# bolcom/serenade

Hardware: AMD Instinct MI355X
Metric: predict_next queries/sec (higher is better)
Workload: dtype u32 ids / i32 accumulators / f64 scores; 1 GPU; BASELINE configs[2]: synthetic 60000000 interactions / 1760000 items, k=1500 m=2500 idf_weighting=2 last_items=4 how_many=21; batch_per_gpu=1048576, query_pool_batches=2, parallelism=query-sharded replicas x1 (no data-path collective), index=csr (built by this library)

## Files before the change

### serenade_amd/csrc/srn_fast.hip

```cpp
#include <hip/hip_runtime.h>

#include <cstdio>
#include <cstdlib>

#include "srn_device.h"
#include "srn_prep.h"
#include "srn_kernels.h"

namespace srn {

#ifndef SRN_FAST_NT
#define SRN_FAST_NT 1
#endif
typedef uint32_t fin_v4u __attribute__((ext_vector_type(4)));
__device__ __forceinline__ void fin_store(uint4* p, const uint4& v) {
#if SRN_FAST_NT
    __builtin_nontemporal_store((fin_v4u{v.x, v.y, v.z, v.w}), reinterpret_cast<fin_v4u*>(p));
#else
    *p = v;
#endif
}
__device__ __forceinline__ uint4 fin_load(const uint4* p) {
#if SRN_FAST_NT
    const fin_v4u v = __builtin_nontemporal_load(reinterpret_cast<const fin_v4u*>(p)); return make_uint4(v.x, v.y, v.z, v.w);
// ... 141 lines not shown
#define SRN_MERGE_ODD 1
#endif
    const uint32_t sb = sa + la, total = la + lb, g = ((total + (1u << lg_nthr) - 1u) >> lg_nthr) | (SRN_MERGE_ODD ? 1u : 0u);
    const uint32_t d0 = min(ttid * g, total), d1 = min(d0 + g, total);
    if (d0 >= d1) return;
    uint32_t lo = d0 > lb ? d0 - lb : 0u, hi = min(d0, la);
    while (lo < hi) {
        const uint32_t mid = (lo + hi) >> 1;
        if (in[sa + mid] > in[sb + d0 - 1 - mid]) lo = mid + 1; else hi = mid;
    }
    const uint32_t* pa = in + sa + lo; const uint32_t* pb = in + sb + (d0 - lo);
    const uint32_t* const ea = in + sb; const uint32_t* const eb = in + sb + lb;
    uint32_t va = pa < ea ? *pa : 0u, vb = pb < eb ? *pb : 0u;
    uint32_t* c = out + sa + d0; uint32_t* const ce = out + sa + d1;
    for (; c < ce; ++c) {
        const bool ta = va > vb;
        *c = max(va, vb);
        const uint32_t* q = (ta ? pa : pb) + 1;
        pa = ta ? q : pa; pb = ta ? pb : q;
        const uint32_t nxt = *q;
        const uint32_t nv = q < (ta ? ea : eb) ? nxt : 0u;
        va = ta ? nv : va; vb = ta ? vb : nv;
    }
}

#ifndef SRN_FAST_FUSED_CUT
#define SRN_FAST_FUSED_CUT 1
#endif
template <int G>
__device__ __forceinline__ uint32_t fast_cut(const uint32_t* F, uint32_t* nbl, uint32_t n, uint32_t NB, uint32_t m, uint32_t k, const uint8_t* wlut, uint32_t* misc, uint32_t tid, uint32_t lane) {
    constexpr int BLOCK = 512;
    const uint32_t NBM = (1u << NB) - 1u;
    const uint32_t g = (n + BLOCK - 1) / BLOCK, o0 = min(tid * g, n), o1 = min(o0 + g, n);
    uint32_t fv[G + 3];
#pragma unroll
    for (int x = 0; x < G + 3; ++x) fv[x] = F[min(o0 + (uint32_t)x, n - 1u)];
    const uint32_t prev0 = o0 > 0u && o0 < o1 ? F[o0 - 1u] >> NB : 0xFFFFFFFFu;
#pragma unroll
    for (int x = 0; x < G + 3; ++x) fv[x] = o0 + (uint32_t)x < n ? fv[x] : 0u;
    {
        uint32_t carry = 0u, carry_r = 0xFFFFFFFFu;
#pragma unroll
        for (int x = G + 2; x >= 0; --x) { const uint32_t r = fv[x] >> NB; carry = r == carry_r ? carry | fv[x] : fv[x]; carry_r = r; fv[x] = carry; }
    }
    uint32_t fmask = 0u, firsts = 0u;
    {
        uint32_t prev = prev0;
#pragma unroll
        for (int x = 0; x < G; ++x) { const bool in = o0 + (uint32_t)x < o1; const uint32_t r = fv[x] >> NB; const bool f1 = in && r != prev; fmask |= f1 ? 1u << x : 0u; firsts += f1; prev = in ? r : prev; }
    }
    uint32_t Call;
    const uint32_t idx0 = block_excl_scan<BLOCK>(firsts, misc + FS_SCAN_A, Call);
    const uint32_t Cm = min(Call, m);
    if (Cm <= k) {
        uint32_t idx = idx0;
#pragma unroll
        for (int x = 0; x < G; ++x) if ((fmask >> x) & 1u) { if (idx < m) nbl[idx] = fv[x]; ++idx; }
        return Cm;
    }
    uint32_t inm = 0u; unsigned long long nmp = 0ull, acc = 0ull;
    {
        uint32_t idx = idx0, nmv[G];
#pragma unroll
        for (int x = 0; x < G; ++x) nmv[x] = (uint32_t)wlut[fv[x] & NBM];
#pragma unroll
        for (int x = 0; x < G; ++x) {
            const bool f1 = (fmask >> x) & 1u, in = f1 && idx < m;
            idx += f1;
            inm |= in ? 1u << x : 0u;
            nmp |= in ? (unsigned long long)nmv[x] << (4 * x) : 0ull;
            acc += in ? 1ull << (4u * nmv[x]) : 0ull;
        }
    }
    uint32_t* cls = misc + FS_CLS;
    {
        uint32_t tot[8];
#pragma unroll
        for (int jj = 0; jj < 4; ++jj) {
            const unsigned long long t = (acc >> (4 * jj)) & 0x000F000F000F000Full;
            tot[2 * jj] = wave_sum((uint32_t)t); tot[2 * jj + 1] = wave_sum((uint32_t)(t >> 32));
        }
        const uint32_t dw = (lane & 3u) * 2u + (lane >> 3);
        uint32_t pick = tot[0];
#pragma unroll
        for (int x = 1; x < 8; ++x) pick = dw == (uint32_t)x ? tot[x] : pick;
        const uint32_t mycnt = lane < 16u ? (pick >> (16u * ((lane >> 2) & 1u))) & 0xFFFFu : 0u;
        if (mycnt) atomicAdd(&cls[lane], mycnt);
    }
    __syncthreads();
    uint32_t nstar, rstar;
    {
        const uint32_t cv = lane < 16u ? cls[lane] : 0u; const uint32_t pre = wave_incl_scan(cv);
        const uint32_t suf = (uint32_t)__builtin_amdgcn_readlane((int)pre, 63) - pre + cv;
        const unsigned long long reach = __ballot(suf >= k);
        nstar = 63u - (uint32_t)__clzll((long long)reach);
        rstar = k - ((uint32_t)__builtin_amdgcn_readlane((int)suf, (int)nstar) - (uint32_t)__builtin_amdgcn_readlane((int)cv, (int)nstar));
    }
    uint32_t mine = 0;
#pragma unroll
    for (int x = 0; x < G; ++x) mine += ((inm >> x) & 1u) && (uint32_t)((nmp >> (4 * x)) & 15ull) == nstar;
    uint32_t tot_star;
    uint32_t before = block_excl_scan<BLOCK>(mine, misc + FS_SCAN_B, tot_star);
    uint32_t sel = 0, tmask = 0;
#pragma unroll
    for (int x = 0; x < G; ++x) {
        const bool in = (inm >> x) & 1u; const uint32_t c = (uint32_t)((nmp >> (4 * x)) & 15ull);
        const bool eq = in && c == nstar, take = in && (c > nstar || (eq && before < rstar));
        tmask |= take ? 1u << x : 0u; sel += take; before += eq;
    }
    const uint32_t inc = wave_incl_scan(sel);
    uint32_t base = 0; if (lane == 63u && inc) base = atomicAdd(&misc[FS_NB], inc);
    uint32_t at = (uint32_t)__builtin_amdgcn_readlane((int)base, 63) + inc - sel;
#pragma unroll
    for (int x = 0; x < G; ++x) if ((tmask >> x) & 1u) nbl[at++] = fv[x];
    return 0xFFFFFFFFu;
}

enum { FM_FUSED = 0, FM_FRONT = 1, FM_BACK = 2 };
template <int WG_PER_CU, bool FRAG, bool WIDE, int MODE = FM_FUSED, bool MID = false, bool BIG = false, bool LONG = false, bool TINY = false>
#ifndef SRN_FAST_WAVES
#define SRN_FAST_WAVES (WG_PER_CU * 2)
#endif
#ifndef SRN_TINY_WAVES
#define SRN_TINY_WAVES 2
#endif
__global__ __launch_bounds__(512, TINY ? SRN_TINY_WAVES : BIG ? 4 : SRN_FAST_WAVES) void vmis_fast_kernel(DeviceIndex ix_arg, LaunchParams p_arg, FastParams f_arg) {
#if SRN_FAST_SMALL
    static_assert(!BIG || MID, "BIG is a form of MID"); static_assert(!LONG || BIG, "LONG is a form of BIG");
    constexpr uint32_t SIDF = BIG ? F_BIG_TOTAL - (F_TOTAL - F_SIDF) : F_SIDF, SATTR = SIDF + 512 * 8;
    constexpr uint32_t MW = (SIDF - F_WORK) / 4;
    __shared__ __attribute__((aligned(16))) char smem[BIG ? F_BIG_TOTAL : F_TOTAL];
#else
    extern __shared__ __attribute__((aligned(16))) char smem[];
#endif
    typedef const __attribute__((address_space(4))) char* KArg;
    const KArg ka = (KArg)__builtin_amdgcn_kernarg_segment_ptr();
    constexpr size_t OFF_P = (sizeof(DeviceIndex) + alignof(LaunchParams) - 1) / alignof(LaunchParams) * alignof(LaunchParams);
    constexpr size_t OFF_F = (OFF_P + sizeof(LaunchParams) + alignof(FastParams) - 1) / alignof(FastParams) * alignof(FastParams);
    const __attribute__((address_space(4))) DeviceIndex& ix = *(const __attribute__((address_space(4))) DeviceIndex*)ka;
    const __attribute__((address_space(4))) LaunchParams& p = *(const __attribute__((address_space(4))) LaunchParams*)(ka + OFF_P);
    const __attribute__((address_space(4))) FastParams& f = *(const __attribute__((address_space(4))) FastParams*)(ka + OFF_F);
    constexpr int BLOCK = 512, NW = 8;
    constexpr int NL = LONG ? (int)F_LONG_LISTS : MID ? (int)F_MID_LISTS : 4;
    constexpr uint32_t SINV = F_SINV;
    static_assert(!MID || MODE == FM_FUSED, "MID: fused form only");
    const uint32_t tid = threadIdx.x, lane = tid & 63u, wave = tid >> 6;
    const unsigned long long lt = (1ull << lane) - 1ull;
    static_assert(!TINY || (MODE == FM_FUSED && !BIG && !FRAG), "TINY: the lean or the MID fused form over an unsharded index");
    if constexpr (TINY) {
        unsigned long long* const a_items = reinterpret_cast<unsigned long long*>(smem + F_W10 + 64); uint32_t* const a_off = reinterpret_cast<uint32_t*>(smem + F_W10 + 64 + 64);
        const uint32_t alen = f.tiny_len;
        if (f.serve == nullptr) {
        if (alen) { if (tid < 8u) a_items[tid] = f.tiny_items[tid]; if (tid == 0u) { a_off[0] = 0u; a_off[1] = alen; } __syncthreads(); }
        if (tid < PREP_LANES) prep_group(ix_arg, alen ? (const uint64_t*)a_items : p.items_flat, alen ? (const uint32_t*)a_off : p.q_off, alen ? 0u : blockIdx.x, tid, p.m, p.max_len,
                                         const_cast<char*>(p.prep) + (size_t)blockIdx.x * p.prep_stride, nullptr, 0u, nullptr);
        __syncthreads();
        }
    }

    uint32_t* misc = (uint32_t*)(smem + F_MISC);
    uint8_t* wlut = (uint8_t*)(smem + F_WLUT);
    uint16_t* w10t = (uint16_t*)(smem + F_W10);
    uint32_t* nbl = (uint32_t*)(smem + F_NBL);
    unsigned long long* ckey = (unsigned long long*)(smem + F_CAND);
    uint32_t* cidx = (uint32_t*)(smem + F_CAND + F_CAND_CAP * 8);
    char* const acc_base = smem + F_HOT;
    uint32_t* hot = (uint32_t*)(smem + F_HOT);
    uint32_t* ikeys = (uint32_t*)(smem + F_TABLE);
    int* iacc = (int*)(smem + F_TABLE + F_TABLE_WORDS * 4);
    uint2* hits = (uint2*)(smem + F_HITS);
    uint32_t* surv = (uint32_t*)(smem + F_SURV);
    constexpr uint32_t SURV_CAP = F_SURV_WORDS - 256u;
    uint32_t* const cls_area = BIG ? (uint32_t*)(smem + SIDF) - 256 : surv + SURV_CAP;
    uint32_t* const dn_area = cls_area - F_M_MAX / 4u;
    uint2* const nb2 = reinterpret_cast<uint2*>(dn_area - F_K_MAX * 2u);
    uint32_t* thist = surv + SURV_CAP;
    auto num_of = [&](uint32_t set) -> uint32_t {
        if constexpr (MID) return (uint32_t)wlut[set & 31u] + (uint32_t)wlut[32u + (set >> 5)];
        else return (uint32_t)wlut[set]; };
    auto w10_of = [&](uint32_t set) -> uint32_t {
        if constexpr (MID) { const uint32_t lo = set & 31u, hi = set >> 5; const uint32_t mp = lo ? (uint32_t)wlut[64u + lo] : (uint32_t)wlut[96u + hi]; return (9u - mp) * ((uint32_t)wlut[lo] + (uint32_t)wlut[32u + hi]); }
        else return (uint32_t)w10t[set]; };

    unsigned long long* tacc = (unsigned long long*)(smem + F_MISC + FS_TACC * 4);
    if (tid < 16u) tacc[tid] = 0ull;
    const bool ticking = p.phase_cycles != nullptr;
    const bool business = (p.flags & SRN_FLAG_BUSINESS_LOGIC) != 0u;
    const uint32_t n_kept = ix.n_kept;
    auto qpos = [&](uint32_t pq) -> uint32_t { return ((wave + NW * (pq >> 6)) << 6) + (pq & 63u); };

    uint32_t* const pre = (uint32_t*)(smem + F_W10 + 64);
    bool have_pre = false;
    { const ItemMeta m0 = f.meta_sample[tid];
      ((double*)(smem + SIDF))[tid] = m0.idf > 0.0 ? m0.idf : 1.0; ((uint8_t*)(smem + SATTR))[tid] = (uint8_t)m0.attr;
      if (tid < 16u) ((double*)(smem + SINV))[tid] = tid < 8u ? f.inv_idf_hot[tid] : f.inv_idf_hi; }
    const bool listed = !MID && MODE == FM_BACK && f.mid_list != nullptr;
    const uint32_t q_end = TINY ? p.nq : LONG ? *f.long_cnt : BIG ? *f.bigq_cnt : MID || listed ? *f.mid_cnt : p.nq;
    const bool ordered = !MID && MODE != FM_FRONT && f.order != nullptr && !listed;
    const uint32_t ox = blockIdx.x & 7u;
    const bool serving = TINY && f.serve != nullptr;
    const uint32_t qi_step = serving ? 0u : ordered ? gridDim.x >> 3 : gridDim.x;
    uint32_t serve_seq = 0u; bool serve_have = false; unsigned long long serve_t0 = 0ull, serve_c0 = 0ull;
    if constexpr (TINY) { if (serving) serve_seq = __atomic_load_n(&(f.serve + blockIdx.x)->done_seq, __ATOMIC_RELAXED); }
    const uint32_t qi_end = ordered ? ord_count(f.order_dups != nullptr ? p.nq - *f.order_dups : p.nq, ox) : q_end;
    for (uint32_t qi = ordered ? blockIdx.x >> 3 : (MODE == FM_FRONT ? f.q_base : 0u) + blockIdx.x; qi < qi_end; qi += qi_step) {
        if constexpr (TINY) {
            if (serving) {
                uint32_t* const sv_flag = reinterpret_cast<uint32_t*>(smem + F_W10 + 64 + 192);
                unsigned long long* const sv_items = reinterpret_cast<unsigned long long*>(smem + F_W10 + 64); uint32_t* const sv_off = reinterpret_cast<uint32_t*>(smem + F_W10 + 64 + 128);
                ServeCtl* const c = f.serve + blockIdx.x;
                __syncthreads();
                if (wave == 0u) {
                    __threadfence_system();
                    uint32_t leave = 0u;
                    if (serve_have && lane == 0u) {
                        const uint32_t cnt = __atomic_load_n(&p.out_counts[blockIdx.x], __ATOMIC_RELAXED);
                        if (cnt & 0x80000000u) { (void)atomicExch(&f.slow_cnt[SC_GENERAL], 0u); (void)atomicExch(&f.slow_cnt[SC_MID], 0u); (void)atomicExch(&f.slow_cnt[SC_BIG_TICKET_LO], 0u); (void)atomicExch(&f.slow_cnt[SC_BIG_TICKET_HI], 0u); }
                        const unsigned long long t_end = wall_clock64();
                        c->stamp[2] = (uint32_t)(t_end - serve_t0); c->stamp[3] = (uint32_t)((unsigned long long)clock64() - serve_c0);
                        __atomic_store_n(&c->count, cnt, __ATOMIC_RELAXED);
                        __atomic_store_n(&c->status, (cnt & 0x80000000u) ? 1u : 0u, __ATOMIC_RELAXED);
                        __threadfence_system();
                        __atomic_store_n(&c->done_seq, serve_seq, __ATOMIC_RELAXED);
                    }
                    const unsigned long long t0 = wall_clock64(), idle = __builtin_nontemporal_load(&c->idle_ticks);
                    uint32_t w = 0u, s_new = 0u, n = 0u;
                    for (;;) {
                        if (lane < 16u) w = __atomic_load_n(reinterpret_cast<const uint32_t*>(c) + lane, __ATOMIC_RELAXED);
                        s_new = (uint32_t)__builtin_amdgcn_readlane((int)w, 0); n = min((uint32_t)__builtin_amdgcn_readlane((int)w, 1), 16u);
                        if (s_new != serve_seq) {
                            uint32_t x = lane >= 4u && lane < 4u + 2u * min(n, 5u) ? w : 0u;
#pragma unroll
                            for (int d = 1; d < 16; d <<= 1) x ^= __shfl_xor(x, d, 16);
                            if ((uint32_t)__builtin_amdgcn_readlane((int)x, 0) == ((uint32_t)__builtin_amdgcn_readlane((int)w, 2) ^ s_new ^ n)) break;
                        }
                        if ((uint32_t)__builtin_amdgcn_readlane((int)w, 3) != 0u || wall_clock64() - t0 > idle) { leave = 1u; break; }
                    }
                    if (!leave) {
                        serve_seq = s_new; serve_have = true; serve_t0 = wall_clock64(); serve_c0 = (unsigned long long)clock64();
                        if (lane >= 4u && lane < 14u) reinterpret_cast<uint32_t*>(sv_items)[lane - 4u] = w;
                        if (n > 5u && lane < 2u * (n - 5u)) reinterpret_cast<uint32_t*>(sv_items)[10u + lane] = __atomic_load_n(reinterpret_cast<const uint32_t*>(c->more) + lane, __ATOMIC_RELAXED);
                        if (lane == 0u) { sv_off[0] = 0u; sv_off[1] = n; p.out_counts[blockIdx.x] = 0x80000002u; c->stamp[0] = (uint32_t)(serve_t0 - t0); }
                    }
                    if (lane == 0u) sv_flag[0] = leave;
                }
                __syncthreads();
                if (sv_flag[0] != 0u) break;
                if (tid < PREP_LANES) prep_group(ix_arg, (const uint64_t*)sv_items, (const uint32_t*)sv_off, 0u, tid, p.m, p.max_len, const_cast<char*>(p.prep) + (size_t)blockIdx.x * p.prep_stride, nullptr, 0u, nullptr);
                __syncthreads();
                if (tid == 0u) c->stamp[1] = (uint32_t)(wall_clock64() - serve_t0);
            }
        }
        const uint32_t q = TINY ? qi : LONG ? f.long_list[qi] : BIG ? f.bigq_list[qi] : MID || listed ? f.mid_list[qi] : ordered ? (uint32_t)f.order[ord_pos(ox, qi)] : qi;
        const uint32_t q_ord_next = ordered && qi + qi_step < qi_end ? (uint32_t)f.order[ord_pos(ox, qi + qi_step)]
                                  : listed && qi + qi_step < qi_end ? f.mid_list[qi + qi_step] : 0xFFFFFFFFu;
#ifndef SRN_MID_PREFETCH
#define SRN_MID_PREFETCH 0
#endif
        const uint32_t q_after = !(MID && SRN_MID_PREFETCH) ? 0xFFFFFFFFu : qi + gridDim.x < q_end ? (BIG ? f.bigq_list : f.mid_list)[qi + gridDim.x] : 0xFFFFFFFFu;
        long long t_prev = ticking ? clock64() : 0;
        FAST_PRIO(FP_REC);
        const char* const rec = p.prep + (size_t)q * p.prep_stride;
        struct { uint32_t U, rmax, xlo, sumw, L, n_staged, cur_attr, unsafe; } hd;
        constexpr uint32_t HW = (uint32_t)sizeof(PrepHead) / 4u;
        struct { uint32_t idx, kept; unsigned long long base; } x0{kNone, 0u, 0ull};
        if (have_pre) {
            auto uni = [&](uint32_t w) -> uint32_t { return (uint32_t)__builtin_amdgcn_readfirstlane((int)pre[w]); };
            hd.U = uni(0); hd.rmax = uni(1); hd.xlo = uni(2); hd.sumw = uni(3); hd.L = uni(6); hd.n_staged = uni(7); hd.cur_attr = uni(16); hd.unsafe = uni(17);
            if (lane < (LONG ? 32u : MID ? 16u : 8u) && lane < hd.L) { const uint32_t* it = pre + HW + 6u * lane; x0.idx = it[0]; x0.kept = it[3]; x0.base = ((unsigned long long)it[5] << 32) | it[4]; }
        } else {
            const PrepHead h0 = *(const PrepHead*)rec;
            hd.U = h0.U; hd.rmax = h0.rmax; hd.xlo = h0.xlo; hd.sumw = h0.sumw; hd.L = h0.L; hd.n_staged = h0.n_staged; hd.cur_attr = h0.cur_attr; hd.unsafe = h0.unsafe;
            if ((MID ? lane < (LONG ? 32u : 16u) && lane < p.max_len : lane < 8u) && lane < hd.L) { const PrepItem pi = ((const PrepItem*)(rec + sizeof(PrepHead)))[lane]; x0.idx = pi.idx; x0.kept = pi.kept; x0.base = pi.base; }
        }
        have_pre = false;
        const uint32_t L = hd.L, n = hd.n_staged, U = hd.U;
        unsigned long long rm = __ballot(x0.kept > 0u);
#ifdef SRN_FAST_EXP_ONELIST
        rm &= 0ull - rm;
#endif
        const uint32_t nr = (uint32_t)__popcll(rm);
        const bool rel = MID || (WIDE && nr > 3u);
        const uint32_t NB = LONG ? F_LONG_NB : MID ? max(nr, 4u) : WIDE && !rel ? 3u : 4u, NBM = (1u << NB) - 1u, base = rel ? hd.xlo : 0u;
        const bool fits = hd.unsafe != 0u ? false : LONG ? L >= 1u && L <= F_LONG_LMAX && L <= p.max_len && hd.sumw <= F_LONG_CLASSES && nr <= F_LONG_LISTS && 2u * n + 8u + F_LONG_RES_WORDS <= MW && hd.rmax - hd.xlo < (1u << (32u - F_LONG_NB))
                        : MID ? L >= 1u && L <= F_MID_LMAX && L <= p.max_len && hd.sumw <= F_MID_CLASSES && nr <= F_MID_LISTS && 2u * n + 8u + 256u <= MW && hd.rmax - hd.xlo < (1u << (32u - NB))
                              : L >= 1u && L <= 8u && L <= p.max_len && hd.sumw <= 15u && nr <= 4u && 2u * n + 8u <= MW && (!rel || hd.rmax - hd.xlo < (1u << 28));
        uint32_t* const xq = MODE == FM_FUSED ? nullptr : f.xchg + (size_t)q * f.xchg_stride;
        if (!fits) {
            if constexpr (MODE == FM_FRONT) { if (tid == 0) xq[0] = 0xFFFFFFFFu; }
            else if (tid == 0) {
                if (hd.unsafe != 0u) f.slow_list[atomicAdd(&f.slow_cnt[SC_GENERAL], 1u)] = q;
                else if (!MID && MODE == FM_FUSED && f.bigq_list != nullptr && L >= 1u && L <= 8u && L <= p.max_len && hd.sumw <= 15u && nr <= 4u && hd.rmax - hd.xlo < (1u << 28) &&
                    2u * n + 8u + 256u <= (F_BIG_TOTAL - (F_TOTAL - F_SIDF) - F_WORK) / 4u) f.bigq_list[atomicAdd(f.bigq_cnt, 1u)] = q;
                else if (!MID && MODE == FM_FUSED && f.mid_list != nullptr && L >= 1u && L <= F_MID_LMAX && L <= p.max_len) f.mid_list[atomicAdd(f.mid_cnt, 1u)] = q;
                else if (!MID && MODE == FM_FUSED && f.long_list != nullptr && L > F_MID_LMAX && L <= F_LONG_LMAX && L <= p.max_len) f.long_list[atomicAdd(f.long_cnt, 1u)] = q;
                else if (MID && !BIG && f.bigq_list != nullptr && L >= 1u && L <= F_MID_LMAX && L <= p.max_len && hd.sumw <= F_MID_CLASSES && nr <= F_MID_LISTS && hd.rmax - hd.xlo < (1u << (32u - NB)) &&
                         2u * n + 8u + 256u <= (F_BIG_TOTAL - (F_TOTAL - F_SIDF) - F_WORK) / 4u) f.bigq_list[atomicAdd(f.bigq_cnt, 1u)] = q;
                else f.slow_list[atomicAdd(&f.slow_cnt[SC_GENERAL], 1u)] = q;
            }
            continue;
        }
        if (n == 0u) { if (tid == 0) { if constexpr (MODE == FM_FRONT) xq[0] = 0u; else p.out_counts[q] = 0u; } continue; }
        uint32_t kp[NL], ps[NL]; const uint32_t* src[NL];
#pragma unroll
        for (int r = 0; r < NL; ++r) {
            const int l = rm ? __ffsll((long long)rm) - 1 : 0;
            kp[r] = rm ? (uint32_t)__builtin_amdgcn_readlane((int)x0.kept, l) : 0u;
            const uint32_t blo = (uint32_t)__builtin_amdgcn_readlane((int)(uint32_t)x0.base, l), bhi = (uint32_t)__builtin_amdgcn_readlane((int)(uint32_t)(x0.base >> 32), l);
            src[r] = ix.post_rank + (((unsigned long long)bhi << 32) | blo);
            ps[r] = (uint32_t)l;
            rm &= rm - 1ull;
        }
        const uint32_t cur_idx = (uint32_t)__builtin_amdgcn_readlane((int)x0.idx, 0);
        const uint32_t cur_attr = hd.cur_attr;
        const uint32_t s1 = kp[0], s2 = s1 + kp[1], s3 = s2 + kp[2];

        uint32_t v[4][5];
        uint32_t K = 0;
        uint32_t pfv[4] = {0u, 0u, 0u, 0u};
        uint32_t xsv[3] = {0u, 0u, 0u};
        if constexpr (MODE == FM_BACK) {
            const uint32_t kv = xq[0];
#pragma unroll
            for (int t = 0; t < 3; ++t) xsv[t] = xq[1u + min(wave * 64u + lane + (uint32_t)t * BLOCK, f.xchg_stride - 2u)];
            K = (uint32_t)__builtin_amdgcn_readfirstlane((int)kv);
        } else {
#pragma unroll
        for (int r = 0; r < 4; ++r)
#pragma unroll
            for (int j = 0; j < 5; ++j) { v[r][j] = 0u; if ((uint32_t)j * BLOCK < kp[r]) v[r][j] = src[r][min(tid + j * BLOCK, kp[r] - 1u)]; }
        }
        __syncthreads();
        FAST_PRIO(FP_FRONT);
        if constexpr (MODE != FM_BACK) {
#pragma unroll
        for (int r = 0; r < 4; ++r)
#pragma unroll
            for (int j = 0; j < 5; ++j) asm volatile("" : "+v"(v[r][j]));
        }
        FAST_TICK(0);
        if (tid < (uint32_t)FS_TACC) misc[tid] = 0;
#ifndef SRN_FAST_EARLY_CLEAR
#define SRN_FAST_EARLY_CLEAR 0
#endif
        const uint32_t clr_lo = (!SRN_FAST_EARLY_CLEAR || MODE == FM_FRONT) ? F_TABLE : (MODE == FM_BACK || nr <= 1u) ? F_HOT : min(F_TABLE, max(F_HOT, (F_WORK + (2u * n + 16u) * 4u + 15u) & ~15u));
        if (SRN_FAST_EARLY_CLEAR && MODE != FM_FRONT) {
            uint4* z = reinterpret_cast<uint4*>(smem);
            for (uint32_t i = clr_lo / 16u + tid; i < F_TABLE / 16u; i += BLOCK) z[i] = make_uint4(0u, 0u, 0u, 0u);
        }
        if constexpr (LONG) {
            if (tid < 32u) {
                uint32_t pr = 0u;
#pragma unroll
                for (int r = 0; r < NL; ++r) pr = tid == (uint32_t)(31 - r) ? ps[r] : pr;
                wlut[tid] = (uint8_t)(L - pr); wlut[32u + tid] = (uint8_t)pr;
            }
        } else
        if constexpr (MID) {
            if (tid < 64u) {
                const uint32_t half = tid >> 5, hs = tid & 31u;
                uint32_t num = 0u, mp = 0u;
                const uint32_t lo = hs ? (uint32_t)__ffs((int)hs) - 1u : 0u;
#pragma unroll
                for (int r = 0; r < 5; ++r) { const uint32_t pr = half ? ps[5 + r] : ps[r]; num += ((hs >> r) & 1u) ? L - pr : 0u; mp = lo == (uint32_t)r ? pr : mp; }
                wlut[tid] = (uint8_t)num; wlut[64u + tid] = (uint8_t)mp;
            }
        } else
        if (tid < (1u << nr)) {
            const uint32_t num = ((tid & 1u) ? L - ps[0] : 0u) + ((tid & 2u) ? L - ps[1] : 0u) + ((tid & 4u) ? L - ps[2] : 0u) + ((tid & 8u) ? L - ps[3] : 0u);
            const uint32_t lo = tid ? (uint32_t)__ffs((int)tid) - 1u : 0u;
            const uint32_t mp = lo == 0u ? ps[0] : lo == 1u ? ps[1] : lo == 2u ? ps[2] : ps[3];
            wlut[tid] = (uint8_t)num; w10t[tid] = (uint16_t)((9u - mp) * num);
        }
        if constexpr (MODE == FM_BACK) {
            if (K == 0xFFFFFFFFu) { if (tid == 0) f.slow_list[atomicAdd(&f.slow_cnt[SC_GENERAL], 1u)] = q; continue; }
            if (K == 0u) { if (tid == 0) p.out_counts[q] = 0u; continue; }
        } else
        if (nr == 1u) {
            K = min(kp[0], p.k);
#pragma unroll
            for (int j = 0; j < 3; ++j) { const uint32_t e = tid + j * BLOCK; if ((uint32_t)j * BLOCK < K && e < K) {
                if constexpr (LONG) nb2[e] = make_uint2(((v[0][j] - base) << NB) | 31u, (uint32_t)((9 - (int)ps[0]) * (int)(L - ps[0])));
                else nbl[e] = ((v[0][j] - base) << NB) | 1u; } }
            __syncthreads();
            FAST_TICK(1);
        } else {
        uint32_t* const B1 = (uint32_t*)(smem + F_WORK); uint32_t* const B0 = B1 + n;
        static_assert(F_WORK == F_NBL, "the m-cut writes the neighbour list in place");
        if constexpr (MID) {
            const uint32_t nlev = nr <= 2u ? 1u : nr <= 4u ? 2u : nr <= 8u ? 3u : nr <= 16u ? 4u : 5u;
            uint32_t* const X = (nlev & 1u) ? B1 : B0; uint32_t* const Y = (nlev & 1u) ? B0 : B1;
            uint32_t pre_r[NL];
            { uint32_t a = 0u;
#pragma unroll
              for (int r = 0; r < NL; ++r) { pre_r[r] = a; a += kp[r]; } }
#pragma unroll
            for (int r = 0; r < 4; ++r)
#pragma unroll
                for (int j = 0; j < 5; ++j) { const uint32_t e = tid + j * BLOCK; if ((uint32_t)j * BLOCK < kp[r] && e < kp[r]) X[pre_r[r] + e] = ((v[r][j] - base) << NB) | (LONG ? 31u - (uint32_t)r : 1u << r); }
#pragma unroll
            for (int b4 = 4; b4 < NL; b4 += 4) {
                if (nr > (uint32_t)b4) {
                    constexpr int R4 = 4;
#pragma unroll
                    for (int r = 0; r < R4; ++r)
#pragma unroll
                        for (int j = 0; j < 5; ++j) { v[r][j] = 0u; if (b4 + r < NL) { if ((uint32_t)j * BLOCK < kp[b4 + r < NL ? b4 + r : 0]) v[r][j] = src[b4 + r < NL ? b4 + r : 0][min(tid + j * BLOCK, kp[b4 + r < NL ? b4 + r : 0] - 1u)]; } }
#pragma unroll
                    for (int r = 0; r < R4; ++r)
#pragma unroll
                        for (int j = 0; j < 5; ++j) asm volatile("" : "+v"(v[r][j]));
#pragma unroll
                    for (int r = 0; r < R4; ++r)
#pragma unroll
                        for (int j = 0; j < 5; ++j) { if (b4 + r < NL) { const int rr = b4 + r < NL ? b4 + r : 0; const uint32_t e = tid + j * BLOCK; if ((uint32_t)j * BLOCK < kp[rr] && e < kp[rr]) X[pre_r[rr] + e] = ((v[r][j] - base) << NB) | (LONG ? 31u - (uint32_t)rr : 1u << rr); } }
                }
            }
            __syncthreads();
            FAST_TICK(1);
            uint32_t len[NL];
#pragma unroll
            for (int r = 0; r < NL; ++r) len[r] = kp[r];
            uint32_t runs = nr; const uint32_t* in = X; uint32_t* out = Y;
#pragma unroll
            for (int lev = 0; lev < (LONG ? 5 : 4); ++lev) {
                if ((uint32_t)lev < nlev) {
                    uint32_t off = 0u, start = 0u;
#pragma unroll
                    for (int j = 0; j < (((NL + (1 << lev) - 1) >> lev) + 1) / 2; ++j) {
                        if (2u * (uint32_t)j < runs) {
                            const uint32_t la = len[2 * j], lb = 2u * (uint32_t)j + 1u < runs ? len[2 * j + 1] : 0u;
                            const uint32_t lg = merge_team(la + lb);
                            merge_pair(in, out, off, la, lb, (tid - start) & 511u, lg);
                            start = (start + (1u << lg)) & 511u; off += la + lb; len[j] = la + lb;
                        }
                    }
                    runs = (runs + 1u) >> 1;
                    uint32_t* const t = const_cast<uint32_t*>(in); in = out; out = t;
                    __syncthreads();
                }
            }
        } else {
        const uint32_t nl = (nr > 1u) + (nr > 2u);
        {
            uint32_t* const d01 = nl == 1u ? B1 : B0; uint32_t* const d2 = nr == 3u ? B1 : B0;
#pragma unroll
            for (int r = 0; r < 4; ++r) {
                uint32_t* const dst = (r < 2 ? d01 : r == 2 ? d2 : B0) + (r == 0 ? 0u : r == 1 ? s1 : r == 2 ? s2 : s3);
#pragma unroll
                for (int j = 0; j < 5; ++j) { const uint32_t e = tid + j * BLOCK; if ((uint32_t)j * BLOCK < kp[r] && e < kp[r]) dst[e] = ((v[r][j] - base) << NB) | (1u << r); }
            }
        }
        __syncthreads();
        FAST_TICK(1);
        if (nr == 2u) { merge_pair(B1, B0, 0u, kp[0], kp[1], tid, merge_team(s2)); __syncthreads(); }
        else if (nr == 3u) { merge_pair(B0, B1, 0u, kp[0], kp[1], tid, merge_team(s2)); __syncthreads(); merge_pair(B1, B0, 0u, s2, kp[2], tid, merge_team(n)); __syncthreads(); }
        else if (nr == 4u) { merge_pair(B0, B1, 0u, kp[0], kp[1], tid, merge_team(s2)); merge_pair(B0, B1, s2, kp[2], kp[3], 511u - tid, merge_team(n - s2)); __syncthreads();
                             merge_pair(B1, B0, 0u, s2, kp[2] + kp[3], tid, merge_team(n)); __syncthreads(); }
        }
        FAST_TICK(3);
        FAST_PRIO(FP_CUT);
        const uint32_t* F = B0; uint32_t* D = B1;
#ifndef SRN_FAST_ROW_PREFETCH
#define SRN_FAST_ROW_PREFETCH 0
#endif
        if constexpr (SRN_FAST_ROW_PREFETCH != 0 && !MID && MODE == FM_FUSED && !FRAG) {
#pragma unroll
            for (int j = 0; j < (SRN_FAST_ROW_PREFETCH == 1 ? 6 : 4); ++j) {
                if ((uint32_t)j * BLOCK < n) {
                    const uint32_t sl = F[min(tid + (uint32_t)j * BLOCK, n - 1u)];
                    const char* a = reinterpret_cast<const char*>(f.row_packed) + (size_t)(base + (sl >> NB)) * 64u;
                    if (SRN_FAST_ROW_PREFETCH == 1) __builtin_amdgcn_global_load_lds((const __attribute__((address_space(1))) void*)a, (__attribute__((address_space(3))) void*)pre, 4, 0, 0);
                    else if (j < 4) pfv[j] = __builtin_nontemporal_load(reinterpret_cast<const uint32_t*>(a));
                }
            }
        }
        if (!MID && SRN_FAST_FUSED_CUT && n <= 6u * BLOCK) {
            const uint32_t kc = fast_cut<6>(F, nbl, n, NB, p.m, p.k, wlut, misc, tid, lane);
            __syncthreads();
            K = kc != 0xFFFFFFFFu ? kc : misc[FS_NB];
            FAST_TICK(2);
        } else {
        uint32_t Call, Cm;
        {
            constexpr int MC_G = 6;
            const uint32_t g = (n + BLOCK - 1) / BLOCK, o0 = min(tid * g, n), o1 = min(o0 + g, n);
            const uint32_t prev0 = o0 > 0u && o0 < o1 ? F[o0 - 1] >> NB : 0xFFFFFFFFu;
            uint32_t firsts = 0, prev = prev0;
            if (g <= (uint32_t)MC_G) {
                uint32_t fv[MC_G];
#pragma unroll
                for (int x = 0; x < MC_G; ++x) fv[x] = F[min(o0 + (uint32_t)x, n - 1u)];
#pragma unroll
                for (int x = 0; x < MC_G; ++x) { const bool in = o0 + (uint32_t)x < o1; const uint32_t r = fv[x] >> NB; firsts += in && r != prev; prev = in ? r : prev; }
            } else
                for (uint32_t o = o0; o < o1; ++o) { const uint32_t r = F[o] >> NB; firsts += r != prev; prev = r; }
            for (uint32_t i = tid; i < min(n, p.m); i += BLOCK) D[i] = 0;
            if (MID && tid < (LONG ? 256u : 64u)) cls_area[tid] = 0u;
            if constexpr (LONG) for (uint32_t i = tid; i < (min(n, p.m) + 3u) / 4u; i += BLOCK) dn_area[i] = 0u;
            uint32_t idx = block_excl_scan<BLOCK>(firsts, misc + FS_SCAN_A, Call);
            prev = prev0;
            if (g <= (uint32_t)MC_G) {
                uint32_t fv[MC_G];
#pragma unroll
                for (int x = 0; x < MC_G; ++x) fv[x] = F[min(o0 + (uint32_t)x, n - 1u)];
#pragma unroll
                for (int x = 0; x < MC_G; ++x) {
                    const bool in = o0 + (uint32_t)x < o1; const uint32_t r = fv[x] >> NB; const bool f1 = in && r != prev;
                    idx += f1; prev = in ? r : prev;
                    if constexpr (LONG) {
                        if (in && idx - 1u < p.m) { if (f1) D[idx - 1u] = fv[x]; atomicAdd(&dn_area[(idx - 1u) >> 2], (uint32_t)wlut[fv[x] & 31u] << (8u * ((idx - 1u) & 3u))); }
                    } else
                    if (in && idx - 1u < p.m) atomicOr(&D[idx - 1u], fv[x]);
                }
            } else
                for (uint32_t o = o0; o < o1; ++o) {
                    const uint32_t v = F[o], r = v >> NB; const bool f1 = r != prev;
                    idx += f1; prev = r;
                    if constexpr (LONG) { if (idx - 1u < p.m) { if (f1) D[idx - 1u] = v; atomicAdd(&dn_area[(idx - 1u) >> 2], (uint32_t)wlut[v & 31u] << (8u * ((idx - 1u) & 3u))); } }
                    else
                    if (idx - 1u < p.m) atomicOr(&D[idx - 1u], v);
                }
            Cm = min(Call, p.m);
        }
        __syncthreads();
        FAST_TICK(2);
        auto dn_of = [&](uint32_t i) -> uint32_t { return (dn_area[i >> 2] >> (8u * (i & 3u))) & 255u; };
        auto w_long = [&](uint32_t slot, uint32_t num) -> uint32_t { return (uint32_t)((9 - (int)(uint32_t)wlut[32u + (slot & 31u)]) * (int)num); };
        if (Cm <= p.k) {
            K = Cm;
            if constexpr (LONG) { for (uint32_t i = tid; i < Cm; i += BLOCK) { const uint32_t dvv = D[i]; nb2[i] = make_uint2(dvv, w_long(dvv, dn_of(i))); } __syncthreads(); }
        } else {
            uint32_t* cls = MID ? cls_area : misc + FS_CLS;
            const uint32_t g = (Cm + BLOCK - 1) / BLOCK, o0 = min(tid * g, Cm), o1 = min(o0 + g, Cm);
            uint32_t dv[5], nmv[5];
#pragma unroll
            for (int x = 0; x < 5; ++x) dv[x] = o0 + x < o1 ? D[o0 + x] : 0u;
#pragma unroll
            for (int x = 0; x < 5; ++x) { if constexpr (LONG) nmv[x] = o0 + x < o1 ? dn_of(o0 + (uint32_t)x) : 0u; else nmv[x] = o0 + x < o1 ? num_of(dv[x] & NBM) : 0u; }
            if constexpr (MID) {
#pragma unroll
                for (int x = 0; x < 5; ++x) if (o0 + x < o1) atomicAdd(&cls[nmv[x]], 1u);
            } else
            {
                unsigned long long acc = 0;
#pragma unroll
                for (int x = 0; x < 5; ++x) acc += o0 + x < o1 ? 1ull << (4u * nmv[x]) : 0ull;
                uint32_t tot[8];
#pragma unroll
                for (int jj = 0; jj < 4; ++jj) {
                    const unsigned long long t = (acc >> (4 * jj)) & 0x000F000F000F000Full;
                    tot[2 * jj] = wave_sum((uint32_t)t); tot[2 * jj + 1] = wave_sum((uint32_t)(t >> 32));
                }
                const uint32_t dw = (lane & 3u) * 2u + (lane >> 3);
                uint32_t pick = tot[0];
#pragma unroll
                for (int x = 1; x < 8; ++x) pick = dw == (uint32_t)x ? tot[x] : pick;
                const uint32_t mycnt = lane < 16u ? (pick >> (16u * ((lane >> 2) & 1u))) & 0xFFFFu : 0u;
                if (mycnt) atomicAdd(&cls[lane], mycnt);
            }
            __syncthreads();
            uint32_t nstar, rstar;
            if constexpr (LONG) {
                const uint4 c4 = reinterpret_cast<const uint4*>(cls)[lane];
                const uint32_t s4 = c4.x + c4.y + c4.z + c4.w, pre4 = wave_incl_scan(s4);
                const uint32_t above = (uint32_t)__builtin_amdgcn_readlane((int)pre4, 63) - pre4;
                const uint32_t suf3 = above + c4.w, suf2 = suf3 + c4.z, suf1 = suf2 + c4.y, suf0 = suf1 + c4.x;
                const unsigned long long reach = __ballot(suf0 >= p.k);
                const int top = 63 - __clzll((long long)reach);
                const uint32_t jsel = suf3 >= p.k ? 3u : suf2 >= p.k ? 2u : suf1 >= p.k ? 1u : 0u;
                const uint32_t sufs = jsel == 3u ? suf3 : jsel == 2u ? suf2 : jsel == 1u ? suf1 : suf0, cnts = jsel == 3u ? c4.w : jsel == 2u ? c4.z : jsel == 1u ? c4.y : c4.x;
                nstar = (uint32_t)__builtin_amdgcn_readlane((int)(4u * lane + jsel), top);
                rstar = p.k - ((uint32_t)__builtin_amdgcn_readlane((int)sufs, top) - (uint32_t)__builtin_amdgcn_readlane((int)cnts, top));
            } else
            {
                const uint32_t cv = (MID || lane < 16u) ? cls[lane] : 0u; const uint32_t pre = wave_incl_scan(cv);
                const uint32_t suf = (uint32_t)__builtin_amdgcn_readlane((int)pre, 63) - pre + cv;
                const unsigned long long reach = __ballot(suf >= p.k);
                nstar = 63u - (uint32_t)__clzll((long long)reach);
                rstar = p.k - ((uint32_t)__builtin_amdgcn_readlane((int)suf, (int)nstar) - (uint32_t)__builtin_amdgcn_readlane((int)cv, (int)nstar));
            }
            uint32_t mine = 0;
#pragma unroll
            for (int x = 0; x < 5; ++x) mine += o0 + x < o1 && nmv[x] == nstar;
            uint32_t tot_star;
            uint32_t before = block_excl_scan<BLOCK>(mine, misc + FS_SCAN_B, tot_star);
            uint32_t sel = 0; bool take[5];
#pragma unroll
            for (int x = 0; x < 5; ++x) {
                const bool in_r = o0 + x < o1, eq = nmv[x] == nstar;
                take[x] = in_r && (nmv[x] > nstar || (eq && before < rstar));
                sel += take[x]; before += in_r && eq;
            }
            const uint32_t inc = wave_incl_scan(sel);
            uint32_t base = 0; if (lane == 63u && inc) base = atomicAdd(&misc[FS_NB], inc);
            uint32_t at = (uint32_t)__builtin_amdgcn_readlane((int)base, 63) + inc - sel;
#pragma unroll
            for (int x = 0; x < 5; ++x) if (take[x]) { if constexpr (LONG) nb2[at++] = make_uint2(dv[x], w_long(dv[x], nmv[x])); else nbl[at++] = dv[x]; }
            __syncthreads();
            K = misc[FS_NB];
        }
        }
        }

        FAST_TICK(4);
        if constexpr (SRN_FAST_ROW_PREFETCH == 2 && !MID && MODE == FM_FUSED && !FRAG) asm volatile("" :: "v"(pfv[0]), "v"(pfv[1]), "v"(pfv[2]), "v"(pfv[3]));
        FAST_PRIO(FP_REQ); FAST_PRIO_X(10);
        if constexpr (MODE == FM_FRONT) {
            if (tid == 0) xq[0] = K;
#pragma unroll
            for (int j = 0; j < 3; ++j) { const uint32_t e = tid + (uint32_t)j * BLOCK; if ((uint32_t)j * BLOCK < K && e < K) xq[1u + e] = nbl[e]; }
            continue;
        }

        uint32_t svr[3]; uint4 rq[3], rq1[3];
        uint32_t wvr[3] = {0u, 0u, 0u};
#pragma unroll
        for (int t = 0; t < 3; ++t) {
            const uint32_t j = wave * 64u + lane + (uint32_t)t * BLOCK;
            if constexpr (MODE == FM_BACK) svr[t] = j < K ? xsv[t] : 0u;
            else if constexpr (LONG) { const uint2 e2 = nb2[K ? min(j, K - 1u) : 0u]; svr[t] = K ? e2.x : 0u; wvr[t] = e2.y; }
            else
            svr[t] = K ? nbl[min(j, K - 1u)] : 0u;
            const size_t r = (MODE == FM_BACK ? j < K : K != 0u) ? (size_t)(base + (svr[t] >> NB)) : (size_t)n_kept;
            rq[t] = *reinterpret_cast<const uint4*>(&f.row_packed[r * (FRAG ? 1 : 4)]); rq1[t] = make_uint4(0u, 0u, 0u, 0u);
        }
        if (((SRN_FAST_PRIO_X) / 10) % 10 != 9) FAST_PRIO(FP_REQ);
        {
            uint4* z = reinterpret_cast<uint4*>(smem + F_HOT);
            for (uint32_t i = tid; i < (clr_lo - F_HOT) / 16u; i += BLOCK) z[i] = make_uint4(0u, 0u, 0u, 0u);
            if (tid < 64u) reinterpret_cast<uint4*>(thist)[tid] = make_uint4(0u, 0u, 0u, 0u);
            if (tid < F_TABLE_WORDS / 4u) { reinterpret_cast<uint4*>(ikeys)[tid] = make_uint4(EMPTY32, EMPTY32, EMPTY32, EMPTY32);
                                            reinterpret_cast<uint4*>(iacc)[tid] = make_uint4(0u, 0u, 0u, 0u); }
        }
        __syncthreads();
        FAST_PRIO(FP_WALK);
        FAST_TICK(8);
        auto add2 = [&](uint32_t wd, uint32_t w) {
            if constexpr (LONG) {
                const bool neg = (int)w < 0; const uint32_t a = wd & 0xFFFFu, b = wd >> 16;
                if (!neg || a < F_SKETCH - F_HOT) atomicAdd((uint32_t*)(acc_base + a), w);
                if (!neg || b < F_SKETCH - F_HOT) atomicAdd((uint32_t*)(acc_base + b), w);
            } else {
            atomicAdd((uint32_t*)(acc_base + (wd & 0xFFFFu)), w); atomicAdd((uint32_t*)(acc_base + (wd >> 16)), w); } };
        constexpr uint32_t INL1 = FRAG ? 6u : 14u, INL2 = FRAG ? 20u : 28u;
        uint32_t cnt3 = 0;
#pragma unroll
        for (int t = 0; t < 3; ++t) {
            const bool m3 = wave * 64u + lane + (uint32_t)t * BLOCK < K && (rq[t].x & 0xFFFFu) > INL1;
            const unsigned long long b3 = __ballot(m3);
            if (m3) nbl[qpos(cnt3 + (uint32_t)__popcll(b3 & lt))] = LONG ? wave * 64u + lane + (uint32_t)t * BLOCK : svr[t];
            cnt3 += (uint32_t)__popcll(b3);
        }
#ifdef SRN_FAST_SUBTICKS
        FAST_TICK(5);
#endif
        if constexpr (!FRAG) {
#pragma unroll
            for (int t = 0; t < 3; ++t) {
                const bool more6 = wave * 64u + lane + (uint32_t)t * BLOCK < K && (rq[t].x & 0xFFFFu) > 6u;
                const size_t r1 = more6 ? (size_t)(base + (svr[t] >> NB)) : (size_t)n_kept;
                rq1[t] = *reinterpret_cast<const uint4*>(&f.row_packed[r1 * 4 + 1]);
            }
        }
        auto tok_slot = [&](uint32_t tok) -> uint32_t { if constexpr (LONG) return nb2[tok].x; else return tok; };
        auto tok_w = [&](uint32_t tok, uint32_t slot) -> uint32_t { if constexpr (LONG) return nb2[tok].y; else return w10_of(slot & NBM); };
        auto q3_load = [&](uint32_t p0, uint32_t& tok, uint32_t& sv, uint32_t& hdr, uint4& c4, uint4& d4, uint32_t& blk) {
            tok = nbl[qpos(min(p0 + lane, cnt3 - 1u))];
            sv = tok_slot(tok);
            if constexpr (FRAG) {
                const uint4 s4 = *reinterpret_cast<const uint4*>(f.row_packed + (size_t)(base + (sv >> NB)));
                hdr = s4.x;
                const uint4* eb = reinterpret_cast<const uint4*>(f.row_ext16) + ((hdr & 0xFFFFu) > 6u ? (size_t)s4.w : (size_t)0);
                c4 = eb[0]; d4 = eb[1]; blk = s4.w + 2u;
            } else {
                const RowQuad* rowp = f.row_packed + (size_t)(base + (sv >> NB)) * 4;
                hdr = *reinterpret_cast<const uint32_t*>(rowp); c4 = *reinterpret_cast<const uint4*>(rowp + 2); d4 = *reinterpret_cast<const uint4*>(rowp + 3); blk = d4.w;
            } };
        uint32_t tk3 = 0, sv3 = 0, hdr3 = 0, blk3 = 0; uint4 c43 = make_uint4(0u, 0u, 0u, 0u), d43 = c43;
        if (cnt3) q3_load(0u, tk3, sv3, hdr3, c43, d43, blk3);
        const uint32_t qn = MID ? q_after : ordered || listed ? q_ord_next : q + gridDim.x;
        const bool park = MID ? q_after != 0xFFFFFFFFu : ordered || listed ? q_ord_next != 0xFFFFFFFFu : qn < p.nq;
        if (wave == 1u && park) {
            const char* const rn = p.prep + (size_t)qn * p.prep_stride + lane * 4u;
            if (lane * 4u < p.prep_stride) __builtin_amdgcn_global_load_lds((const __attribute__((address_space(1))) void*)rn, (__attribute__((address_space(3))) void*)pre, 4, 0, 0);
            if (256u + lane * 4u < min(p.prep_stride, 320u)) __builtin_amdgcn_global_load_lds((const __attribute__((address_space(1))) void*)(rn + 256), (__attribute__((address_space(3))) void*)(pre + 64), 4, 0, 0);
        }
#pragma unroll
        for (int t = 0; t < 3; ++t) {
            if (wave * 64u + (uint32_t)t * BLOCK < K) {
                const bool act = wave * 64u + lane + (uint32_t)t * BLOCK < K;
                const uint32_t w = LONG ? wvr[t] : w10_of(svr[t] & NBM), len = rq[t].x & 0xFFFFu;
                if constexpr (FRAG) { if (act) { add2(rq[t].y, w); add2(rq[t].z, w); if (len <= 6u) add2(rq[t].w, w); } }
                else {
                if (act) { add2(rq[t].y, w); add2(rq[t].z, w); add2(rq[t].w, w); }
                if (act && len > 6u) { add2(rq1[t].x, w); add2(rq1[t].y, w); add2(rq1[t].z, w); add2(rq1[t].w, w); }
                }
            }
        }
        auto add_tail = [&](uint32_t p0, uint32_t tok, uint32_t sv, uint32_t hdr, const uint4& c4, const uint4& d4, uint32_t blk) {
            const bool act = p0 + lane < cnt3;
            const uint32_t len = hdr & 0xFFFFu, w = tok_w(tok, sv);
            const bool more = FRAG ? true : len > 30u;
            if constexpr (FRAG) {
                if (act) { add2(c4.x, w); add2(c4.y, w); add2(c4.z, w); add2(c4.w, w); }
                if (act && len > 12u) { add2(d4.x, w); add2(d4.y, w); add2(d4.z, w); add2(d4.w, w); }
            } else if (act) {
                add2(c4.x, w); add2(c4.y, w); add2(c4.z, w); add2(c4.w, w);
                add2(d4.x, w); add2(d4.y, w); add2(d4.z, w);
                if (len <= 30u) add2(d4.w, w);
            }
            for (uint32_t t8 = INL2; __ballot(act && more && t8 < len) != 0ull; t8 += 8u) {
                if (act && more && t8 < len) {
                    const uint4 e4 = reinterpret_cast<const uint4*>(f.row_ext16)[(size_t)blk + ((t8 - INL2) >> 3)];
                    add2(e4.x, w); add2(e4.y, w); add2(e4.z, w); add2(e4.w, w);
                }
            } };
#ifdef SRN_FAST_SUBTICKS
        FAST_TICK(6);
#endif
        FAST_PRIO_X(1);
        if (cnt3) add_tail(0u, tk3, sv3, hdr3, c43, d43, blk3);
        for (uint32_t p0 = 64u; p0 < cnt3; p0 += 64u) { uint32_t tk, sv, hdr, blk; uint4 c4, d4; q3_load(p0, tk, sv, hdr, c4, d4, blk); add_tail(p0, tk, sv, hdr, c4, d4, blk); }
#ifdef SRN_FAST_SUBTICKS
        FAST_TICK(7);
#endif
        __syncthreads();
        FAST_PRIO(FP_HARV);
        FAST_TICK(9);
        uint32_t t32m1; uint32_t floor_b;
        {
            const uint32_t e = lane * NW + wave;
            uint32_t v = hot[e];
            if (F_REP_ITEMS && e < F_REP_ITEMS) {
                const uint4* rp = reinterpret_cast<const uint4*>(hot + F_DIRECT + e * F_REP);
                const uint4 a = rp[0], b = rp[1];
                v = a.x + a.y + a.z + a.w + b.x + b.y + b.z + b.w;
            }
            if (!SRN_FAST_PHANTOM_OOR || BIG)
            for (uint32_t i = tid; i < F_PHANTOM_WORDS; i += BLOCK) ((uint32_t*)(smem + F_PHANTOM))[i] = 0u;
            bool valid = (LONG ? (int)v > 0 : v != 0u) && e != cur_idx;
            double x = 0.0; uint32_t tie = 0;
            tie = f.meta_sample[tid].id_rank;
            if (business) valid = valid && business_ok(cur_attr, (uint32_t)((const uint8_t*)(smem + SATTR))[tid]);
            if (valid) x = ((const double*)(smem + SIDF))[tid] * (double)v;
            const uint32_t k32 = (uint32_t)((unsigned long long)__double_as_longlong(x) >> 32);
            {
                uint32_t vv = k32, third = 0;
#pragma unroll
                for (int t = 0; t < 3; ++t) {
                    const uint32_t mx = wave_max(vv);
                    third = mx;
                    const unsigned long long bal = __ballot(vv == mx);
                    if ((int)lane == __ffsll((long long)bal) - 1) vv = 0;
                }
                for (uint32_t t = 3u; t < ((p.how_many + 7u) >> 3); ++t) {
                    const uint32_t mx = wave_max(vv);
                    third = mx;
                    const unsigned long long bal = __ballot(vv == mx);
                    if ((int)lane == __ffsll((long long)bal) - 1) vv = 0;
                }
// ... 532 lines not shown
```

Measured before the change: 53.81 million queries/s.

## Sort posting runs by length and use a chain merge for uneven four-run queries

For the non-MID fast path, the up to four posting runs are now sorted by length with a small sorting network, recording their original slot indices. Shorter runs load with fewer rounds per thread, and the class bits are remapped to keep the weight tables correct. When one run dominates, the four-way merge becomes a chain that merges the short runs first, so less data moves through the merge levels. It adds sorting and index bookkeeping on the scalar path and makes buffer placement more complex.

After: 53.40 million queries/s. About the same (-0.8%).

```diff
diff --git a/serenade_amd/csrc/srn_fast.hip b/serenade_amd/csrc/srn_fast.hip
--- a/serenade_amd/csrc/srn_fast.hip
+++ b/serenade_amd/csrc/srn_fast.hip
@@ -467,6 +467,8 @@
         }
         if (n == 0u) { if (tid == 0) { if constexpr (MODE == FM_FRONT) xq[0] = 0u; else p.out_counts[q] = 0u; } continue; }
         uint32_t kp[NL], ps[NL]; const uint32_t* src[NL];
+        uint32_t rnum = 0u, pspk = 0u;
+        if constexpr (MID) {
 #pragma unroll
         for (int r = 0; r < NL; ++r) {
             const int l = rm ? __ffsll((long long)rm) - 1 : 0;
@@ -476,11 +478,33 @@
             ps[r] = (uint32_t)l;
             rm &= rm - 1ull;
         }
+        } else {
+            const uint32_t rm0 = (uint32_t)rm;
+            uint32_t key[4];
+#pragma unroll
+            for (int r = 0; r < 4; ++r) {
+                const int l = rm ? __ffsll((long long)rm) - 1 : 0;
+                key[r] = rm ? ((uint32_t)__builtin_amdgcn_readlane((int)x0.kept, l) << 3) | (uint32_t)l : 0u;
+                ps[r] = 0u; pspk |= (uint32_t)l << (3 * r);
+                rm &= rm - 1ull;
+            }
+            auto cx = [&](int a, int b) { const uint32_t hi = max(key[a], key[b]), lo = min(key[a], key[b]); key[a] = hi; key[b] = lo; };
+            cx(0, 1); cx(2, 3); cx(0, 2); cx(1, 3); cx(1, 2);
+#pragma unroll
+            for (int i = 0; i < 4; ++i) {
+                const int l = (int)(key[i] & 7u);
+                kp[i] = key[i] >> 3;
+                const uint32_t blo = (uint32_t)__builtin_amdgcn_readlane((int)(uint32_t)x0.base, l), bhi = (uint32_t)__builtin_amdgcn_readlane((int)(uint32_t)(x0.base >> 32), l);
+                src[i] = ix.post_rank + (((unsigned long long)bhi << 32) | blo);
+                rnum |= (uint32_t)__popc(rm0 & ((1u << l) - 1u)) << (2 * i);
+            }
+        }
         const uint32_t cur_idx = (uint32_t)__builtin_amdgcn_readlane((int)x0.idx, 0);
         const uint32_t cur_attr = hd.cur_attr;
-        const uint32_t s1 = kp[0], s2 = s1 + kp[1], s3 = s2 + kp[2];
 
         uint32_t v[4][5];
+        auto rounds = [](int r) constexpr -> int { return MID ? 5 : r == 2 ? 4 : r == 3 ? 3 : 5; };
+        static_assert(MID || ((MW - 8u) / 2u / 3u <= 4u * BLOCK && (MW - 8u) / 2u / 4u <= 3u * BLOCK), "the load rounds of the lean form's shorter runs");
         uint32_t K = 0;
         uint32_t pfv[4] = {0u, 0u, 0u, 0u};
         uint32_t xsv[3] = {0u, 0u, 0u};
@@ -493,7 +517,7 @@
 #pragma unroll
         for (int r = 0; r < 4; ++r)
 #pragma unroll
-            for (int j = 0; j < 5; ++j) { v[r][j] = 0u; if ((uint32_t)j * BLOCK < kp[r]) v[r][j] = src[r][min(tid + j * BLOCK, kp[r] - 1u)]; }
+            for (int j = 0; j < 5; ++j) { v[r][j] = 0u; if (j < rounds(r) && (uint32_t)j * BLOCK < kp[r]) v[r][j] = src[r][min(tid + j * BLOCK, kp[r] - 1u)]; }
         }
         __syncthreads();
         FAST_PRIO(FP_FRONT);
@@ -501,7 +525,7 @@
 #pragma unroll
         for (int r = 0; r < 4; ++r)
 #pragma unroll
-            for (int j = 0; j < 5; ++j) asm volatile("" : "+v"(v[r][j]));
+            for (int j = 0; j < 5; ++j) if (j < rounds(r)) asm volatile("" : "+v"(v[r][j]));
         }
         FAST_TICK(0);
         if (tid < (uint32_t)FS_TACC) misc[tid] = 0;
@@ -532,9 +556,10 @@
             }
         } else
         if (tid < (1u << nr)) {
-            const uint32_t num = ((tid & 1u) ? L - ps[0] : 0u) + ((tid & 2u) ? L - ps[1] : 0u) + ((tid & 4u) ? L - ps[2] : 0u) + ((tid & 8u) ? L - ps[3] : 0u);
+            const uint32_t p0 = pspk & 7u, p1 = (pspk >> 3) & 7u, p2 = (pspk >> 6) & 7u, p3 = (pspk >> 9) & 7u;
+            const uint32_t num = ((tid & 1u) ? L - p0 : 0u) + ((tid & 2u) ? L - p1 : 0u) + ((tid & 4u) ? L - p2 : 0u) + ((tid & 8u) ? L - p3 : 0u);
             const uint32_t lo = tid ? (uint32_t)__ffs((int)tid) - 1u : 0u;
-            const uint32_t mp = lo == 0u ? ps[0] : lo == 1u ? ps[1] : lo == 2u ? ps[2] : ps[3];
+            const uint32_t mp = (pspk >> (3u * lo)) & 7u;
             wlut[tid] = (uint8_t)num; w10t[tid] = (uint16_t)((9u - mp) * num);
         }
         if constexpr (MODE == FM_BACK) {
@@ -606,22 +631,30 @@
                 }
             }
         } else {
-        const uint32_t nl = (nr > 1u) + (nr > 2u);
+#ifndef SRN_FAST_CHAIN_DIV
+#define SRN_FAST_CHAIN_DIV 0
+#endif
+        const uint32_t t2 = kp[3] + kp[2], t3 = t2 + kp[1];
+        const uint32_t chain = SRN_FAST_CHAIN_DIV >= 0 && nr == 4u && t2 + t3 + (SRN_FAST_CHAIN_DIV > 0 ? n / (uint32_t)(SRN_FAST_CHAIN_DIV > 0 ? SRN_FAST_CHAIN_DIV : 1) : 0u) < n ? 1u : 0u;
+        const uint32_t tree = nr + chain;
         {
-            uint32_t* const d01 = nl == 1u ? B1 : B0; uint32_t* const d2 = nr == 3u ? B1 : B0;
+            const uint32_t o3 = tree == 5u ? 0u : n, o1 = t2 + (tree == 2u ? 0u : n), o0 = t3 + (tree == 4u ? n : 0u);
 #pragma unroll
             for (int r = 0; r < 4; ++r) {
-                uint32_t* const dst = (r < 2 ? d01 : r == 2 ? d2 : B0) + (r == 0 ? 0u : r == 1 ? s1 : r == 2 ? s2 : s3);
-#pragma unroll
-                for (int j = 0; j < 5; ++j) { const uint32_t e = tid + j * BLOCK; if ((uint32_t)j * BLOCK < kp[r] && e < kp[r]) dst[e] = ((v[r][j] - base) << NB) | (1u << r); }
+                uint32_t* const dst = B1 + (r == 0 ? o0 : r == 1 ? o1 : r == 2 ? o3 + kp[3] : o3);
+#pragma unroll
+                for (int j = 0; j < 5; ++j) { const uint32_t e = tid + j * BLOCK; if (j < rounds(r) && (uint32_t)j * BLOCK < kp[r] && e < kp[r]) dst[e] = ((v[r][j] - base) << NB) | (1u << ((rnum >> (2 * r)) & 3u)); }
             }
         }
         __syncthreads();
         FAST_TICK(1);
-        if (nr == 2u) { merge_pair(B1, B0, 0u, kp[0], kp[1], tid, merge_team(s2)); __syncthreads(); }
-        else if (nr == 3u) { merge_pair(B0, B1, 0u, kp[0], kp[1], tid, merge_team(s2)); __syncthreads(); merge_pair(B1, B0, 0u, s2, kp[2], tid, merge_team(n)); __syncthreads(); }
-        else if (nr == 4u) { merge_pair(B0, B1, 0u, kp[0], kp[1], tid, merge_team(s2)); merge_pair(B0, B1, s2, kp[2], kp[3], 511u - tid, merge_team(n - s2)); __syncthreads();
-                             merge_pair(B1, B0, 0u, s2, kp[2] + kp[3], tid, merge_team(n)); __syncthreads(); }
+        if (tree >= 4u) {
+            if (tree == 5u) merge_pair(B1, B0, 0u, kp[3], kp[2], tid, merge_team(t2));
+            else { merge_pair(B0, B1, 0u, kp[3], kp[2], tid, merge_team(t2)); merge_pair(B0, B1, t2, kp[1], n - t3, 511u - tid, merge_team(n - t2)); }
+            __syncthreads();
+        }
+        if (tree == 3u || tree == 5u) { merge_pair(B0, B1, 0u, t2, kp[1], tid, merge_team(t3)); __syncthreads(); }
+        { const uint32_t la = tree == 4u ? t2 : t3; merge_pair(B1, B0, 0u, la, n - la, tid, merge_team(n)); __syncthreads(); }
         }
         FAST_TICK(3);
         FAST_PRIO(FP_CUT);
```
